# RoyiAvital/QuadraticProgramSolver

Hardware: AMD Instinct MI355X
Metric: ADMM iterations/sec (higher is better)
Workload: dtype f64

## Files before the change

quadraticprogramsolver_amd/csrc/k_loop.hip:

```cpp
#include <cstdlib>

#include "qps_kernels.h"
#include "wave_reduce.h"
#include <hip/hip_ext.h>

namespace qps {

namespace {

template <typename T> __device__ __forceinline__ T wave_sum(T v) { return wave_sum_all(v); }
__device__ __forceinline__ unsigned long long absbits(double v) { return (unsigned long long)__double_as_longlong(fabs(v)); }
__device__ __forceinline__ unsigned long long wave_max_u64(unsigned long long v) {
#pragma unroll
    for (int o = 32; o > 0; o >>= 1) { unsigned long long t = __shfl_xor(v, o, 64); v = t > v ? t : v; }
    return v;
}

template <typename T, int RB, int TRI, int THREADS>
__global__ __launch_bounds__(THREADS) void k_gemv_rows(const T* __restrict__ S, int64_t ld, const T* __restrict__ v,
                                                   T* __restrict__ out, const T* __restrict__ out0, T alpha, T beta,
                                                   int r0, int c0, int c1, BatchStride bs) {
    using V = typename VecOf<T>::type;
    if (bs.active && !bs.active[blockIdx.y]) return;
    S += (int64_t)blockIdx.y * bs.mat; v += (int64_t)blockIdx.y * bs.vin; out += (int64_t)blockIdx.y * bs.vout;
// ... 29 lines not shown
                acc[i] += ok ? ap[e] * vp[e] : T(0);
            }
        }
    }
    __shared__ T red[THREADS / 64][RB];
#pragma unroll
    for (int i = 0; i < RB; ++i) acc[i] = wave_sum(acc[i]);
    if ((tid & 63) == 0) {
#pragma unroll
        for (int i = 0; i < RB; ++i) red[tid >> 6][i] = acc[i];
    }
    __syncthreads();
    if (tid < RB) {
        T s = T(0);
#pragma unroll
        for (int w = 0; w < THREADS / 64; ++w) s += red[w][tid];
        T r = alpha * s;
        if (beta != T(0)) r += beta * out0[rb + tid];
        out[rb + tid] = r;
    }
}

constexpr int GC_RT = 32;
template <typename T>
__global__ __launch_bounds__(256) void k_gemv_cols(const T* __restrict__ S, int64_t ld, const T* __restrict__ va,
                                                   const T* __restrict__ vb, T ca, T cb, T* __restrict__ part,
                                                   int64_t part_ld, int ncols) {
    using V = typename VecOf<T>::type;
    constexpr int VN = VecOf<T>::N;
    const int c = (blockIdx.x * 256 + threadIdx.x) * VN;
    if (c >= ncols) return;
    const int rt = blockIdx.y;
    const int rbase = rt * GC_RT;
    T acc[VN];
#pragma unroll
    for (int e = 0; e < VN; ++e) acc[e] = T(0);
    const T* Sp = S + (int64_t)rbase * ld + c;
#pragma unroll 8
    for (int i = 0; i < GC_RT; ++i) {
        T w = ca * va[rbase + i];
        if (vb) w += cb * vb[rbase + i];
        typedef T NV __attribute__((ext_vector_type(VN)));
        const NV a = __builtin_nontemporal_load(reinterpret_cast<const NV*>(Sp + (int64_t)i * ld));
#pragma unroll
        for (int e = 0; e < VN; ++e) acc[e] += a[e] * w;
    }
    V o;
    T* op = reinterpret_cast<T*>(&o);
#pragma unroll
    for (int e = 0; e < VN; ++e) op[e] = acc[e];
    *reinterpret_cast<V*>(part + (int64_t)rt * part_ld + c) = o;
}

template <typename T>
__global__ __launch_bounds__(256) void k_colsum(const T* __restrict__ part, int64_t part_ld, int ntiles,
                                                const T* __restrict__ a0, T s0, const T* __restrict__ a1, T s1,
                                                T* __restrict__ out, int ncols, BatchStride bs) {
    using V = typename VecOf<T>::type;
    constexpr int VN = VecOf<T>::N;
    if (bs.active && !bs.active[blockIdx.y]) return;
    part += (int64_t)blockIdx.y * bs.mat; out += (int64_t)blockIdx.y * bs.vout;
    if (a0) a0 += (int64_t)blockIdx.y * bs.vin;
    if (a1) a1 += (int64_t)blockIdx.y * bs.vin;
    constexpr int COLS = 128 / (int)sizeof(T);
    constexpr int CL = COLS / VN;
    constexpr int TL = 256 / CL;
    const int cl = threadIdx.x % CL, tl = threadIdx.x / CL;
    const int c = blockIdx.x * COLS + cl * VN;
    T acc[VN];
#pragma unroll
    for (int e = 0; e < VN; ++e) acc[e] = T(0);
    if (c < ncols) {
        int t = tl;
        for (; t + 7 * TL < ntiles; t += 8 * TL) {
            V v[8];
#pragma unroll
            for (int j = 0; j < 8; ++j) v[j] = *reinterpret_cast<const V*>(part + (int64_t)(t + TL * j) * part_ld + c);
#pragma unroll
            for (int j = 0; j < 8; ++j) {
                const T* vp = reinterpret_cast<const T*>(&v[j]);
#pragma unroll
                for (int e = 0; e < VN; ++e) acc[e] += vp[e];
            }
        }
        for (; t < ntiles; t += TL) {
            const V v = *reinterpret_cast<const V*>(part + (int64_t)t * part_ld + c);
            const T* vp = reinterpret_cast<const T*>(&v);
#pragma unroll
            for (int e = 0; e < VN; ++e) acc[e] += vp[e];
        }
    }
    __shared__ T red[TL][COLS + 1];
#pragma unroll
    for (int e = 0; e < VN; ++e) red[tl][cl * VN + e] = acc[e];
    __syncthreads();
    constexpr int PL = 256 / COLS;
    static_assert(TL % PL == 0 && (PL == 16 || PL == 8), "slab lanes per output");
    const int o = threadIdx.x / PL, pl = threadIdx.x % PL;
    T s = T(0);
#pragma unroll
    for (int k = 0; k < TL / PL; ++k) s += red[pl * (TL / PL) + k][o];
    s = (PL == 16) ? row16_sum_last(s) : oct_sum_all(s);
    const int oc = blockIdx.x * COLS + o;
    if (pl == PL - 1 && oc < ncols) {
        T r = s;
        if (a0) r += s0 * a0[oc];
        if (a1) r += s1 * a1[oc];
        out[oc] = r;
    }
}

template <typename T>
__global__ __launch_bounds__(256) void k_admm_update(int NP, int MP, const T* __restrict__ xx, const T* __restrict__ zz,
                                                     T* __restrict__ x, T* __restrict__ xp, T* __restrict__ z,
                                                     T* __restrict__ zp, T* __restrict__ y, const T* __restrict__ l,
                                                     const T* __restrict__ u, T alpha, T rho) {
    const int i = blockIdx.x * 256 + threadIdx.x;
    const T alpha1 = T(1) - alpha, rho1 = T(1) / rho;
    if (i < NP) {
        const T xo = x[i];
        xp[i] = xo;
        x[i] = alpha * xx[i] + alpha1 * xo;
    }
    if (i < MP) {
        const T zo = z[i], yo = y[i], zt = zz[i];
        zp[i] = zo;
        T t = alpha * zt + alpha1 * zo + rho1 * yo;
        const T lo = l[i], hi = u[i];
        const T zn = t > hi ? hi : (t < lo ? lo : t);
        z[i] = zn;
        y[i] = yo + rho * (alpha * zt + alpha1 * zo - zn);
    }
}

template <typename T>
__global__ __launch_bounds__(256) void k_check_norms(int n, int m, const T* __restrict__ Ax, const T* __restrict__ Px,
                                                     const T* __restrict__ Aty, const T* __restrict__ q,
                                                     const T* __restrict__ x, const T* __restrict__ xp,
                                                     const T* __restrict__ z, const T* __restrict__ zp,
                                                     unsigned long long* __restrict__ slots, int dual_only, BatchStride bs) {
    if (bs.active && !bs.active[blockIdx.y]) return;
    {
        const int64_t on = (int64_t)blockIdx.y * bs.vin, om = (int64_t)blockIdx.y * bs.vout;
        Ax += om; z += om; zp += om; Px += on; Aty += on; q += on; x += on; xp += on; slots += (int64_t)blockIdx.y * 16;
    }
    unsigned long long v[9];
#pragma unroll
    for (int k = 0; k < 9; ++k) v[k] = 0ull;
    for (int i = blockIdx.x * 256 + threadIdx.x; i < max(n, m); i += gridDim.x * 256) {
        if (i < m && !dual_only) {
            const double ax = (double)Ax[i], zi = (double)z[i];
            v[0] = max(v[0], absbits((double)(Ax[i] - z[i])));
            v[2] = max(v[2], absbits(ax));
            v[3] = max(v[3], absbits(zi));
            v[8] = max(v[8], absbits((double)(z[i] - zp[i])));
        }
        if (i < n) {
            v[1] = max(v[1], absbits((double)(Px[i] + q[i] + Aty[i])));
            v[4] = max(v[4], absbits((double)Px[i]));
            v[5] = max(v[5], absbits((double)Aty[i]));
            v[6] = max(v[6], absbits((double)q[i]));
            if (!dual_only) v[7] = max(v[7], absbits((double)(x[i] - xp[i])));
        }
    }
#pragma unroll
    for (int k = 0; k < 9; ++k) {
        v[k] = wave_max_u64(v[k]);
        if ((threadIdx.x & 63) == 0 && v[k] != 0ull) atomicMax(&slots[k], v[k]);
    }
}

__device__ __forceinline__ double jmax(double a, double b) { return (isnan(a) || isnan(b)) ? (double)NAN : (a > b ? a : b); }

__global__ void k_check_decide(const unsigned long long* __restrict__ slots, double* __restrict__ res, CheckScalars cs,
                               const double* __restrict__ rho_arr, const double* __restrict__ rhorho_arr,
                               const int* __restrict__ active) {
    if (threadIdx.x != 0) return;
    const int b = blockIdx.x;
    if (active && !active[b]) return;
    slots += (int64_t)b * 16; res += (int64_t)b * 8;
    if (rho_arr) { cs.rho = rho_arr[b]; cs.rhorho = rhorho_arr[b]; cs.convFlag = 1; }
    double nv[9];
    for (int k = 0; k < 9; ++k) nv[k] = __longlong_as_double((long long)slots[k]);
    const double MIN_VAL_RHO = 1e-3, MAX_VAL_RHO = 1e6;
    const double normResPrim = nv[0], normResDual = nv[1];
    const double maxNormPrim = jmax(nv[2], nv[3]);
    const double maxNormDual = jmax(jmax(nv[4], nv[5]), nv[6]);
    double rhorho = cs.rhorho;
    if (cs.adptRho) {
        const double numeratorVal = normResPrim * maxNormDual;
        const double denominatorVal = normResDual * maxNormPrim;
        const double t = cs.rho * sqrt(numeratorVal / denominatorVal);
        rhorho = t > MAX_VAL_RHO ? MAX_VAL_RHO : (t < MIN_VAL_RHO ? MIN_VAL_RHO : t);
    }
    const double epsPrim = cs.epsAbs + cs.epsRel * maxNormPrim;
    const double epsDual = cs.epsAbs + cs.epsRel * maxNormDual;
    int flag = cs.convFlag;
    if ((normResPrim < epsPrim) && (normResDual < epsDual)) flag = 3;
    if ((nv[7] <= cs.epsAdmm) && (nv[8] <= cs.epsAdmm)) flag = 2;
    res[0] = normResPrim; res[1] = normResDual; res[2] = maxNormPrim; res[3] = maxNormDual;
    res[4] = rhorho; res[5] = (double)flag; res[6] = nv[7]; res[7] = nv[8];
}

template <typename T> __global__ void k_fill(T* p, int64_t n, T v) {
    int64_t i = (int64_t)blockIdx.x * 256 + threadIdx.x;
    if (i < n) p[i] = v;
}
template <typename T> __global__ void k_convert(const double* __restrict__ s, T* __restrict__ d, int64_t n) {
    int64_t i = (int64_t)blockIdx.x * 256 + threadIdx.x;
    if (i < n) d[i] = (T)s[i];
}
template <typename T> __global__ void k_convert_back(const T* __restrict__ s, double* __restrict__ d, int64_t n) {
    int64_t i = (int64_t)blockIdx.x * 256 + threadIdx.x;
    if (i < n) d[i] = (double)s[i];
}

}

static int env_int(const char* name, int dflt) { const char* e = getenv(name); return e ? atoi(e) : dflt; }

template <typename T, int RB, int TH>
static void gemv_rows_launch(hipStream_t st, const T* S, int64_t ld, const T* v, T* out, const T* out0, T alpha, T beta, int r0,
                             int r1, int c0, int c1, int tri, BatchStride bs) {
    dim3 grid((r1 - r0 + RB - 1) / RB, bs.count);
#define QPS_GR(TRI) hipLaunchKernelGGL((k_gemv_rows<T, RB, TRI, TH>), grid, dim3(TH), 0, st, S, ld, v, out, out0, alpha, beta, r0, c0, c1, bs)
    if (tri == 0) QPS_GR(0); else if (tri == 1) QPS_GR(1); else QPS_GR(2);
#undef QPS_GR
}

template <typename T>
void gemv_rows(hipStream_t st, const T* S, int64_t ld, const T* v, T* out, const T* out0, T alpha, T beta, int r0, int r1,
               int c0, int c1, int tri, BatchStride bs) {
    if (r1 <= r0) return;
    static const int wide_th = env_int("QPS_GEMV_WIDE_THREADS", 512);
    static const int wide_rb = env_int("QPS_GEMV_WIDE_RB", 2);
    const bool wide = (c1 - c0) >= 4 * 256 * VecOf<T>::N;
    if (!wide) { gemv_rows_launch<T, 4, 256>(st, S, ld, v, out, out0, alpha, beta, r0, r1, c0, c1, tri, bs); return; }
#define QPS_W(RB, TH) gemv_rows_launch<T, RB, TH>(st, S, ld, v, out, out0, alpha, beta, r0, r1, c0, c1, tri, bs)
    if (wide_th == 512) { if (wide_rb == 4) QPS_W(4, 512); else QPS_W(VecOf<T>::N == 2 ? 2 : 4, 512); }
    else if (wide_th == 256) { if (wide_rb == 4) QPS_W(4, 256); else QPS_W(VecOf<T>::N == 2 ? 2 : 4, 256); }
    else { if (wide_rb == 4) QPS_W(4, 1024); else QPS_W(VecOf<T>::N == 2 ? 2 : 4, 1024); }
#undef QPS_W
}

int gemv_cols_tiles(int nrows) { return (nrows + GC_RT - 1) / GC_RT; }

template <typename T>
int gemv_cols_partial(hipStream_t st, const T* S, int64_t ld, const T* va, const T* vb, T ca, T cb, T* part,
                      int64_t part_ld, int nrows, int ncols) {
    constexpr int VN = VecOf<T>::N;
    const int tiles = gemv_cols_tiles(nrows);
    if (tiles == 0) return 0;
    dim3 grid((ncols + 256 * VN - 1) / (256 * VN), tiles), block(256);
    hipLaunchKernelGGL((k_gemv_cols<T>), grid, block, 0, st, S, ld, va, vb, ca, cb, part, part_ld, ncols);
    return tiles;
}

template <typename T>
void colsum(hipStream_t st, const T* part, int64_t part_ld, int ntiles, const T* a0, T s0, const T* a1, T s1, T* out,
            int ncols, BatchStride bs) {
    constexpr int cols_wg = 128 / (int)sizeof(T);
    if (g_launch_timing.start) {
        const LaunchTiming lt = g_launch_timing;
        g_launch_timing = LaunchTiming();
        hipExtLaunchKernelGGL((k_colsum<T>), dim3((ncols + cols_wg - 1) / cols_wg, bs.count), dim3(256), 0, st, lt.start, lt.stop, 0, part, part_ld, ntiles, a0, s0, a1, s1, out, ncols, bs);
        return;
    }
    hipLaunchKernelGGL((k_colsum<T>), dim3((ncols + cols_wg - 1) / cols_wg, bs.count), dim3(256), 0, st, part, part_ld, ntiles, a0, s0, a1, s1, out, ncols, bs);
}

template <typename T>
void admm_update(hipStream_t st, int NP, int MP, const T* xx, const T* zz, T* x, T* xp, T* z, T* zp, T* y, const T* l,
                 const T* u, T alpha, T rho) {
    const int N = NP > MP ? NP : MP;
    hipLaunchKernelGGL((k_admm_update<T>), dim3((N + 255) / 256), dim3(256), 0, st, NP, MP, xx, zz, x, xp, z, zp, y, l, u, alpha, rho);
}

template <typename T>
void check_convergence(hipStream_t st, int n, int m, const T* Ax, const T* Px, const T* Aty, const T* q, const T* x,
                       const T* xp, const T* z, const T* zp, unsigned long long* scratch, double* res_dev, CheckScalars cs,
                       int dual_only, BatchStride bs, const double* rho_arr, const double* rhorho_arr) {
    if (!dual_only) (void)hipMemsetAsync(scratch, 0, 16 * sizeof(unsigned long long) * bs.count, st);
    const int N = n > m ? n : m;
    int blocks = (N + 255) / 256;
    if (blocks > 1024) blocks = 1024;
    if (blocks < 1) blocks = 1;
    hipLaunchKernelGGL((k_check_norms<T>), dim3(blocks, bs.count), dim3(256), 0, st, n, m, Ax, Px, Aty, q, x, xp, z, zp, scratch, dual_only, bs);
    hipLaunchKernelGGL(k_check_decide, dim3(bs.count), dim3(64), 0, st, scratch, res_dev, cs, rho_arr, rhorho_arr, bs.active);
}

template <typename T> void fill(hipStream_t st, T* p, int64_t n, T v) {
    if (n <= 0) return;
    hipLaunchKernelGGL((k_fill<T>), dim3((unsigned)((n + 255) / 256)), dim3(256), 0, st, p, n, v);
}
template <typename T> void convert_copy(hipStream_t st, const double* src, T* dst, int64_t n) {
    if (n <= 0) return;
    hipLaunchKernelGGL((k_convert<T>), dim3((unsigned)((n + 255) / 256)), dim3(256), 0, st, src, dst, n);
}
template <typename T> void convert_back(hipStream_t st, const T* src, double* dst, int64_t n) {
    if (n <= 0) return;
    hipLaunchKernelGGL((k_convert_back<T>), dim3((unsigned)((n + 255) / 256)), dim3(256), 0, st, src, dst, n);
}

#define INST(T)                                                                                                              \
    template void gemv_rows<T>(hipStream_t, const T*, int64_t, const T*, T*, const T*, T, T, int, int, int, int, int, BatchStride); \
    template int gemv_cols_partial<T>(hipStream_t, const T*, int64_t, const T*, const T*, T, T, T*, int64_t, int, int);      \
    template void colsum<T>(hipStream_t, const T*, int64_t, int, const T*, T, const T*, T, T*, int, BatchStride);            \
    template void admm_update<T>(hipStream_t, int, int, const T*, const T*, T*, T*, T*, T*, T*, const T*, const T*, T, T);   \
    template void check_convergence<T>(hipStream_t, int, int, const T*, const T*, const T*, const T*, const T*, const T*,    \
                                       const T*, const T*, unsigned long long*, double*, CheckScalars, int, BatchStride,     \
                                       const double*, const double*);                                                        \
    template void fill<T>(hipStream_t, T*, int64_t, T);                                                                      \
    template void convert_copy<T>(hipStream_t, const double*, T*, int64_t);                                                  \
    template void convert_back<T>(hipStream_t, const T*, double*, int64_t);
INST(double)
INST(float)
#undef INST

}
```

quadraticprogramsolver_amd/csrc/k_pass.hip:

```cpp
#include "k_pass_kernel.h"

namespace qps {

static int pass_threads() {
    static int th = [] { const char* e = getenv("QPS_PASS_THREADS"); int v = e ? atoi(e) : 512; return v == 1024 ? 1024 : 512; }();
    return th;
}

template <typename T> static int pass_threads_for(int NP) { return (pass_threads() == 1024 || NP > 8 * 512 * VecOf<T>::N) ? 1024 : 512; }
template <typename T> int apass_max_np() { return 8 * 1024 * VecOf<T>::N; }

template <typename T> int apass_plan(int NP, int MP, int* rows_per_wg, int count) {
    if (NP > apass_max_np<T>() || MP <= 0) { *rows_per_wg = 0; return 0; }
    const int R = 4;
    static const int total_env = [] { const char* e = getenv("QPS_PASS_WGS"); return e ? atoi(e) : 0; }();
    const int kc1 = NP <= pass_threads_for<T>(NP) * VecOf<T>::N;
    const int total = total_env > 0 ? total_env : ((kc1 && count > 1) ? 1024 : 256);
    const int target = count >= total ? 1 : total / (count < 1 ? 1 : count);
    int rpw = (MP + target - 1) / target;
    rpw = ((rpw + R - 1) / R) * R;
    *rows_per_wg = rpw;
    return (MP + rpw - 1) / rpw;
}

template <typename T, int TH>
void apass_th(hipStream_t st, bool check, const T* A, int64_t ld, int NP, int MP, const T* xx, const T* x_old, T* x_new, T* z,
              T* y, const T* l, const T* u, T alpha, T rho, T* part, T* part2, int64_t part_ld, unsigned long long* slots,
              PassBatch pb) {
    int rpw = 0;
    const int G = apass_plan<T>(NP, MP, &rpw, pb.count);
    pb.slabs = G;
    const int chunk = TH * VecOf<T>::N;
    const int kc = (NP + chunk - 1) / chunk;
#define QPS_PASS(KC, R, RC) launch_pass<T, TH, KC, R, RC, 0>(st, check, G, A, ld, NP, MP, rpw, xx, x_old, x_new, z, y, l, u, alpha, rho, part, part2, part_ld, slots, pb)
    if (TH == 512) {
        if (kc <= 1) QPS_PASS(1, 4, 4);
        else if (kc <= 2) QPS_PASS(2, 4, 4);
        else if (kc <= 4) QPS_PASS(4, 4, 2);
        else QPS_PASS(8, 2, 1);
    } else {
        if (kc <= 1) QPS_PASS(1, 4, 4);
        else if (kc <= 2) QPS_PASS(2, 4, 2);
        else if (kc <= 4) QPS_PASS(4, 2, 1);
        else QPS_PASS(8, 1, 1);
    }
#undef QPS_PASS
}

template <typename T>
void apass(hipStream_t st, bool check, const T* A, int64_t ld, int NP, int MP, const T* xx, const T* x_old, T* x_new, T* z,
           T* y, const T* l, const T* u, T alpha, T rho, T* part, T* part2, int64_t part_ld, unsigned long long* slots,
           PassBatch pb) {
    if (pass_threads_for<T>(NP) == 1024) apass_th<T, 1024>(st, check, A, ld, NP, MP, xx, x_old, x_new, z, y, l, u, alpha, rho, part, part2, part_ld, slots, pb);
    else apass_th<T, 512>(st, check, A, ld, NP, MP, xx, x_old, x_new, z, y, l, u, alpha, rho, part, part2, part_ld, slots, pb);
}

#define INST(T)                                                                                                            \
    template int apass_max_np<T>();                                                                                        \
    template int apass_plan<T>(int, int, int*, int);                                                                       \
    template void apass<T>(hipStream_t, bool, const T*, int64_t, int, int, const T*, const T*, T*, T*, T*, const T*, const T*, \
                           T, T, T*, T*, int64_t, unsigned long long*, PassBatch);
INST(double)
INST(float)
#undef INST

}
```

quadraticprogramsolver_amd/csrc/qps_dense.hip:

```cpp
#include <memory>

#include "dense_chol.h"
#include "qps_batch.h"
#include "qps_internal.h"
#include "qps_kernels.h"
#include "qps_polish.h"

namespace qps {
namespace {

template <typename T> struct DenseSolver : SolverBase {
    int NP = 0, MP = 0;
    T *A = nullptr, *P = nullptr, *q = nullptr, *l = nullptr, *u = nullptr;
    T *PI = nullptr, *AA = nullptr, *M = nullptr, *S = nullptr, *tmp = nullptr, *dinv = nullptr; int* fail = nullptr;
    T *x = nullptr, *xp = nullptr, *z = nullptr, *zp = nullptr, *y = nullptr, *xx = nullptr, *zz = nullptr, *tt = nullptr, *yv = nullptr;
    T *part = nullptr, *part2 = nullptr, *sw_part = nullptr, *Ax = nullptr, *Px = nullptr, *Aty = nullptr;
    T* At = nullptr; void* small_out = nullptr; void* small_out_host = nullptr; bool small_ok = false;
    StreamLease lease; Arena arena;
    double* stage_mat = nullptr; int64_t stage_mat_count = 0;
    int pass_slabs = 0, pass_rpw = 0;
    unsigned long long* scratch = nullptr; double* res_dev = nullptr; double* res_host = nullptr; double* stage = nullptr;
    bool have_AA = false, factor_valid = false; double fac_rho = 0, fac_sigma = 0; int fac_nb = 0;
    int nb = 2048; int part_tiles = 0; int num_factorizations = 0;
    unsigned long long* pub = nullptr; unsigned* abort_dev = nullptr; unsigned sweep_epoch = 0; bool blocked_off = false, fac_premul = false;
    bool use_blocked() const { return !blocked_off && trsv_blocked_supported<T>(NP, nb); }
    struct IterGraph { int count; const void* xa; double rho, sigma, alpha; int nb; hipGraphExec_t exec; };
    std::vector<IterGraph> graphs;
    bool graphs_disabled = false;
    void drop_graphs() { for (auto& gr : graphs) (void)hipGraphExecDestroy(gr.exec); graphs.clear(); }
    hipGraphExec_t iter_graph(int count, T* xa, T* xb, double rho, double sigma, double alpha) {
        for (auto& gr : graphs) if (gr.count == count && gr.xa == xa && gr.rho == rho && gr.sigma == sigma && gr.alpha == alpha && gr.nb == nb) return gr.exec;
        if (graphs_disabled) return nullptr;
        if (graphs.size() >= 8) drop_graphs();
        hipGraph_t graph = nullptr; hipGraphExec_t exec = nullptr;
        if (hipStreamBeginCapture(st, hipStreamCaptureModeThreadLocal) != hipSuccess) { (void)hipGetLastError(); graphs_disabled = true; return nullptr; }
        for (int k = 0; k < count; ++k) {
            colsum<T>(st, part, NP, pass_slabs, xa, (T)sigma, q, T(-1), tt, NP);
            sweeps();
            apass<T>(st, false, A, NP, NP, MP, xx, xa, xb, z, y, l, u, (T)alpha, (T)rho, part, part2, NP, scratch);
            std::swap(xa, xb);
        }
        if (hipStreamEndCapture(st, &graph) != hipSuccess || graph == nullptr) { (void)hipGetLastError(); graphs_disabled = true; return nullptr; }
        const hipError_t e = hipGraphInstantiate(&exec, graph, nullptr, nullptr, 0);
        (void)hipGraphDestroy(graph);
        if (e != hipSuccess) { (void)hipGetLastError(); graphs_disabled = true; return nullptr; }
        graphs.push_back({count, xa, rho, sigma, alpha, nb, exec});
        return exec;
    }
    int prof_iter = 0;
    int sample_lvl(int slot) const { return (prof.level == 1 && prof_iter % 50 == slot) ? 1 : 2; }
    int cat_atw, cat_colsum, cat_fwd, cat_bwd, cat_ax, cat_upd, cat_chk, cat_pass, cat_passchk, cat_sweep, cat_xsum, cat_small;

    DenseSolver(int dev, int64_t n_, int64_t m_, int dt) {
        device = dev; n = n_; m = m_; dtype = dt;
        HIPC(hipSetDevice(device));
        NP = roundup(n, 64); MP = roundup(m, 64);
        const int64_t nn = (int64_t)NP * NP;
        part_tiles = gemv_cols_tiles(MP);
        pass_slabs = apass_plan<T>(NP, MP, &pass_rpw);
        const int slabs = std::max(std::max(part_tiles, pass_slabs), 1);
        small_ok = admm_small_supported<T>((int)n, (int)m, NP, MP);
        stage_mat_count = std::max((int64_t)n * n, (int64_t)m * n);
        if (stage_mat_count > ((int64_t)1 << 20)) stage_mat_count = 0;
        auto layout = [&](Arena& ar) {
            A = ar.take<T>((int64_t)MP * NP); P = ar.take<T>(nn); q = ar.take<T>(NP); l = ar.take<T>(MP); u = ar.take<T>(MP);
            PI = ar.take<T>(nn); AA = ar.take<T>(nn); M = ar.take<T>(nn); S = ar.take<T>(nn); tmp = ar.take<T>(nn);
            dinv = ar.take<T>((int64_t)(NP / 64) * 4096); fail = ar.take<int>(4);
            x = ar.take<T>(NP); xp = ar.take<T>(NP); xx = ar.take<T>(NP); tt = ar.take<T>(NP); yv = ar.take<T>(NP);
            z = ar.take<T>(MP); zp = ar.take<T>(MP); y = ar.take<T>(MP); zz = ar.take<T>(MP);
            part = ar.take<T>((int64_t)slabs * NP);
            part2 = ar.take<T>((int64_t)slabs * NP);
            sw_part = ar.take<T>((int64_t)std::max(sweep_fused_slabs<T>(NP), 1) * NP);
            Ax = ar.take<T>(MP); Px = ar.take<T>(NP); Aty = ar.take<T>(NP);
            scratch = ar.take<unsigned long long>(16); res_dev = ar.take<double>(16);
            pub = ar.take<unsigned long long>(trsv_blocked_pub_words<T>(NP));
            abort_dev = reinterpret_cast<unsigned*>(res_dev + 14);
            stage = ar.take<double>((int64_t)NP + 2 * (int64_t)MP + 64);
            if (small_ok) { At = ar.take<T>((int64_t)NP * MP); small_out = ar.take<double>(32); }
            if (stage_mat_count > 0) stage_mat = ar.take<double>(stage_mat_count);
        };
        layout(arena);
        st = prof.st = lease.acquire(device, arena.planned());
        HandleResources& res = lease.res;
        char* const recycled = res.block; res.block = nullptr;
        arena.commit(st, recycled, res.block_bytes);
        layout(arena);
        res_host = reinterpret_cast<double*>(res.pinned);
        small_out_host = small_ok ? reinterpret_cast<char*>(res.pinned) + 16 * sizeof(double) : nullptr;
        const double s = sizeof(T);
        cat_atw = prof.category("gemv_cols(A'w)", s * ((double)m * n + m + n));
        cat_colsum = prof.category("colsum(rhs)", s * ((double)part_tiles * n + 3.0 * n));
        cat_fwd = prof.category("trsv_forward", s * ((double)n * (n + 1) / 2 + 2.0 * n));
        cat_bwd = prof.category("trsv_backward", s * ((double)n * (n + 1) / 2 + 2.0 * n));
        cat_ax = prof.category("gemv_rows(Ax~)", s * ((double)m * n + m + n));
        cat_upd = prof.category("admm_update", s * (3.0 * n + 7.0 * m));
        cat_chk = prof.category("check_convergence", s * (2.0 * m * n + (double)n * n + 4.0 * n + 4.0 * m));
        cat_pass = prof.category("apass(fused A-pass)", s * ((double)m * n + 3.0 * n + 6.0 * m));
        cat_passchk = prof.category("apass(check variant)", s * ((double)m * n + 4.0 * n + 6.0 * m));
        cat_sweep = prof.category("sweeps(fused fwd+bwd, triangle read once)", s * ((double)n * (n + 1) / 2 + 2.0 * n + (double)sweep_fused_slabs<T>(NP) * n));
        cat_xsum = prof.category("colsum(x~ slabs)", s * ((double)sweep_fused_slabs<T>(NP) * n + n));
        cat_small = prof.category("admm_small(whole loop in one launch; bytes per iteration)", s * ((double)m * n + (double)n * n) + s * (6.0 * n + 10.0 * m));
    }
    ~DenseSolver() override {
        (void)hipSetDevice(device);
        (void)hipStreamSynchronize(st);
        trsv_blocked_forget_stream(device, st);
        drop_graphs();
        prof.release_events();
        lease.res.block = arena.base; lease.res.block_bytes = arena.bytes; arena.base = nullptr;
    }

    void upload_vec(const double* h, T* d, int64_t count) { HIPC(upload_staged<T>(st, stage, h, d, count)); }
    void download_vec(const T* d, double* h, int64_t count) { HIPC(download_staged<T>(st, stage, d, h, count)); }
    void upload_matrix(const double* h, int64_t ldh, int rows, int cols, T* d, int64_t ldd) {
        if (rows <= 0 || cols <= 0) return;
        if (stage_mat && (int64_t)rows * cols <= stage_mat_count) {
            HIPC(hipMemcpy2DAsync(stage_mat, sizeof(double) * (size_t)rows, h, sizeof(double) * (size_t)ldh, sizeof(double) * (size_t)rows, (size_t)cols, hipMemcpyHostToDevice, st));
            import_colmajor<T>(st, stage_mat, rows, rows, cols, d, ldd);
            HIPC(hipStreamSynchronize(st));
            return;
        }
        upload_matrix_panels<T>(st, device, h, ldh, rows, cols, d, ldd);
    }

    DenseChol<T> chol() const { return {st, (int)n, NP, MP, P, A, PI, AA, M, S, tmp, dinv, fail}; }
    void factorize(double rho, double sigma, bool rebuild_all) {
        const bool rebuild = rebuild_all || !have_AA;
        const DenseChol<T> c = chol();
        factor_valid = false;
        c.form(sigma, rho, rebuild, rebuild);
        have_AA = true;
        c.factor(nb, 1, use_blocked());
        char ctx[128]; snprintf(ctx, sizeof ctx, "rho=%g, sigma=%g; factorisation #%d of this handle", rho, sigma, ++num_factorizations);
        int f = 0;
        c.check("P + sigma I + rho A'A", ctx, &f);
        factor_valid = true; fac_rho = rho; fac_sigma = sigma; fac_nb = nb; fac_premul = use_blocked();
    }
    bool sweep_gave_up(bool fetched = false) {
        if (!fac_premul) return false;
        unsigned* h = reinterpret_cast<unsigned*>(res_host + 14);
// ... 13 lines not shown
            chol().sweeps(nb, tt, yv, xx, sw_part, BatchStride(), {&prof, cat_sweep, sample_lvl(13), cat_xsum, sample_lvl(21), cat_fwd, cat_bwd, 2});
            return;
        }
        if (sweep_epoch >= 0xfffffff0u) {
            HIPC(hipMemsetAsync(pub, 0, sizeof(unsigned long long) * (size_t)trsv_blocked_pub_words<T>(NP), st));
            sweep_epoch = 0;
        }
        TrsvBlockedPair gate(device, st);
        { ProfLaunchScope ps(prof, cat_fwd, sample_lvl(13)); trsv_blocked<T>(st, false, S, NP, NP, nb, tt, yv, pub, ++sweep_epoch, abort_dev); }
        { ProfLaunchScope ps(prof, cat_bwd, sample_lvl(21)); trsv_blocked<T>(st, true, S, NP, NP, nb, yv, xx, pub, ++sweep_epoch, abort_dev); }
    }
    void linear_solve(double rho, double sigma) {
        {
            ProfScope ps(prof, cat_atw, 1);
            gemv_cols_partial<T>(st, A, NP, z, y, (T)rho, T(-1), part, NP, MP, NP);
        }
        {
            ProfScope ps(prof, cat_colsum, 2);
            colsum<T>(st, part, NP, part_tiles, x, (T)sigma, q, T(-1), tt, NP);
        }
        sweeps();
        {
            ProfScope ps(prof, cat_ax, 2);
            gemv_rows<T>(st, A, NP, xx, zz, nullptr, T(1), T(0), 0, MP, 0, NP, 0);
        }
    }

    void solve(double* xh, const qps_params& p, qps_info* info) override {
        HIPC(hipSetDevice(device));
        blocked_off = false;
        int gave_up = 0; double t_lost = 0;
        const double t_begin = now_s();
        while (solve_once(xh, p, info)) {
            ++gave_up; t_lost = now_s() - t_begin;
            const int lvl = prof.level; prof.reset(); prof.level = lvl;
        }
        if (info) { info->sweepGaveUp = gave_up; info->cgExplicit = 0; info->tLoop += t_lost; }
    }
    bool solve_once(double* xh, const qps_params& p, qps_info* info) {
        if (p.linsys != QPS_LINSYS_AUTO && p.linsys != QPS_LINSYS_CHOLESKY)
            throw QpsError(QPS_ERR_UNSUPPORTED, "dense handles offer QPS_LINSYS_CHOLESKY only (qps_create_csc with dense_path = 0 for the CG and the sparse L D L' plugins)");
        const double t0 = now_s();
        nb = pick_nb<T>(p.trsvBlock, NP);
        double rho = p.rho, sigma = p.sigma; const double alpha = p.alpha;
        const double epsAdmm = std::fmin(p.epsAbs, p.epsRel) * 1e-2;
        int convFlag = QPS_CONV_NUM_ITR;
        const bool reuse = p.reuseFactor && factor_valid && fac_rho == rho && fac_sigma == sigma && fac_nb == nb && fac_premul == use_blocked();
        if (!reuse) factorize(rho, sigma, !p.reuseFactor || !have_AA || fac_sigma != sigma);
        upload_vec(xh, x, n);
        HIPC(hipMemsetAsync(xp, 0, sizeof(T) * NP, st));
        HIPC(hipMemsetAsync(z, 0, sizeof(T) * std::max(MP, 64), st));
        HIPC(hipMemsetAsync(y, 0, sizeof(T) * std::max(MP, 64), st));
        HIPC(hipMemsetAsync(zp, 0, sizeof(T) * std::max(MP, 64), st));
        HIPC(hipStreamSynchronize(st));
        const double t1 = now_s();
        double rhorho = rho;
        int ii = 0, nref = 0; double tref = 0, resP = NAN, resD = NAN;
        auto finish = [&](int iterations, double t_end, int variant) {
            PolishReport pr;
            if (p.polish) polish_dense<T>(st, n, m, NP, MP, P, A, q, l, u, y, x, part, p, &pr);
            download_vec(x, xh, n);
            if (info) {
                info->convFlag = convFlag; info->iterations = iterations; info->numRefactor = nref; info->cgIterations = 0;
                info->rhoFinal = rho; info->rhoProposed = rhorho; info->resPrim = resP; info->resDual = resD;
                info->tSetup = t1 - t0; info->tLoop = t_end - t1; info->tRefactor = tref;
                info->polishFlag = pr.flag; info->polishIterations = pr.minresIterations; info->tPolish = pr.seconds;
                info->trsvBlock = nb; info->sweepVariant = variant;
            }
            return false;
        };
        if (small_ok && p.loopVariant == 0 && (NP + nb - 1) / nb == 1) {
            transpose_small<T>(st, A, NP, MP, At);
            int it = 0;
            while (it < p.numIterations) {
                {
                    ProfScope ps(prof, cat_small, 1);
                    admm_small<T>(st, (int)n, (int)m, NP, MP, it, p.numIterations, p.numItrConv, p.adptRho, rho, rhorho, sigma, alpha, p.epsAbs,
                                  p.epsRel, epsAdmm, p.fctrRho, A, At, P, S, q, l, u, x, xp, z, y, small_out);
                }
                HIPC(hipMemcpyAsync(small_out_host, small_out, admm_small_out_bytes(), hipMemcpyDeviceToHost, st));
                HIPC(hipStreamSynchronize(st));
                prof.harvest();
                int last = 0, flag = 1, need = 0; double r8[8];
                admm_small_read(small_out_host, &last, &flag, &need, r8);
                it = last; convFlag = flag; rhorho = r8[4];
                if (!std::isnan(r8[0]) || !std::isnan(r8[1])) { resP = r8[0]; resD = r8[1]; }
                if (flag != QPS_CONV_NUM_ITR) break;
                if (need && it < p.numIterations) {
                    rho = rhorho; ++nref;
                    const double ta = now_s();
                    factorize(rho, sigma, false);
                    tref += now_s() - ta;
                }
            }
            return finish(it, now_s(), 4);
        }
        const bool fused = pass_slabs > 0 && p.loopVariant != 1;
        int rhs_slabs = 0;
        static const int graph_env = [] { const char* e = getenv("QPS_GRAPH"); return e ? atoi(e) : -1; }();
        const bool use_graph = fused && prof.level == 0 && p.numItrConv >= 3 && !fac_premul && (graph_env >= 0 ? graph_env != 0 : NP <= 2048);
        for (ii = 1; ii <= p.numIterations; ++ii) {
            bool changed = false;
            if (p.adptRho && ((rhorho * p.fctrRho < rho) || (rhorho > p.fctrRho * rho))) {
                rho = rhorho; ++nref; changed = true;
                const double ta = now_s();
                factorize(rho, sigma, false);
                tref += now_s() - ta;
            }
            const bool check = (ii % p.numItrConv == 0);
            if (use_graph && !changed && !check && rhs_slabs == pass_slabs) {
                int run = std::min(p.numItrConv - ii % p.numItrConv, p.numIterations - ii + 1) & ~1;
                hipGraphExec_t ge = run >= 2 ? iter_graph(run, x, xp, rho, sigma, alpha) : nullptr;
                if (ge) {
                    HIPC(hipGraphLaunch(ge, st));
                    ii += run - 1;
                    continue;
                }
            }
            if (!fused) {
                linear_solve(rho, sigma);
                {
                    ProfScope ps(prof, cat_upd, 2);
                    admm_update<T>(st, NP, MP, xx, zz, x, xp, z, zp, y, l, u, (T)alpha, (T)rho);
                }
                if (check) {
                    ProfScope ps(prof, cat_chk, 2);
                    gemv_rows<T>(st, A, NP, x, Ax, nullptr, T(1), T(0), 0, MP, 0, NP, 0);
                    gemv_rows<T>(st, P, NP, x, Px, nullptr, T(1), T(0), 0, NP, 0, NP, 0);
                    gemv_cols_partial<T>(st, A, NP, y, nullptr, T(1), T(0), part, NP, MP, NP);
                    colsum<T>(st, part, NP, part_tiles, nullptr, T(0), nullptr, T(0), Aty, NP);
                    CheckScalars cs{p.epsAbs, p.epsRel, epsAdmm, rho, rhorho, p.adptRho, convFlag};
                    check_convergence<T>(st, (int)n, (int)m, Ax, Px, Aty, q, x, xp, z, zp, scratch, res_dev, cs);
                }
            } else {
                if (changed && rhs_slabs > 0) {
                    ProfScope ps(prof, cat_atw, 2);
                    rhs_slabs = gemv_cols_partial<T>(st, A, NP, z, y, (T)rho, T(-1), part, NP, MP, NP);
                }
                prof_iter = ii;
                {
                    ProfLaunchScope ps(prof, cat_colsum, sample_lvl(29));
                    colsum<T>(st, part, NP, rhs_slabs, x, (T)sigma, q, T(-1), tt, NP);
                }
                sweeps();
                if (check) HIPC(hipMemsetAsync(scratch, 0, 16 * sizeof(unsigned long long), st));
                {
                    const int lvl = (prof.level == 1 && (check || ii % 50 != 38)) ? 3 : 1;
                    ProfLaunchScope ps(prof, check ? cat_passchk : cat_pass, lvl);
                    apass<T>(st, check, A, NP, NP, MP, xx, x, xp, z, y, l, u, (T)alpha, (T)rho, part, part2, NP, scratch);
                }
                std::swap(x, xp);
                rhs_slabs = pass_slabs;
                if (check) {
                    ProfScope ps(prof, cat_chk, 2);
                    colsum<T>(st, part2, NP, pass_slabs, nullptr, T(0), nullptr, T(0), Aty, NP);
                    gemv_rows<T>(st, P, NP, x, Px, nullptr, T(1), T(0), 0, NP, 0, NP, 0);
                    CheckScalars cs{p.epsAbs, p.epsRel, epsAdmm, rho, rhorho, p.adptRho, convFlag};
                    check_convergence<T>(st, (int)n, (int)m, Ax, Px, Aty, q, x, xp, z, zp, scratch, res_dev, cs, 1);
                }
            }
            if (check) {
                HIPC(hipMemcpyAsync(res_host, res_dev, 15 * sizeof(double), hipMemcpyDeviceToHost, st));
                HIPC(hipStreamSynchronize(st));
                prof.harvest();
                if (sweep_gave_up(true)) return true;
                resP = res_host[0]; resD = res_host[1]; rhorho = res_host[4]; convFlag = (int)res_host[5];
                if (convFlag != QPS_CONV_NUM_ITR) break;
            }
        }
        HIPC(hipStreamSynchronize(st));
        prof.harvest();
        if (sweep_gave_up()) return true;
        return finish(ii > p.numIterations ? p.numIterations : ii, now_s(), sweep_variant());
    }
    void polish(double* xh, const double* yh, const qps_params& p, qps_polish_report* rep) override {
        HIPC(hipSetDevice(device));
        upload_vec(xh, x, n); upload_vec(yh, y, m);
        PolishReport pr;
        polish_dense<T>(st, n, m, NP, MP, P, A, q, l, u, y, x, part, p, &pr);
        download_vec(x, xh, n);
        if (rep) {
            rep->flag = pr.flag; rep->refinements = pr.refinements; rep->minresIterations = pr.minresIterations;
            rep->numActiveLower = pr.numLower; rep->numActiveUpper = pr.numUpper; rep->reserved0 = 0; rep->relres = pr.relres; rep->seconds = pr.seconds;
        }
    }
    void get_dual(double* zh, double* yh) override {
        HIPC(hipSetDevice(device));
        if (zh) download_vec(z, zh, m);
        if (yh) download_vec(y, yh, m);
    }
    void linsys_init(double rho, double sigma, int linsys, int nbreq) override {
        HIPC(hipSetDevice(device));
        if (linsys != QPS_LINSYS_AUTO && linsys != QPS_LINSYS_CHOLESKY) throw QpsError(QPS_ERR_UNSUPPORTED, "dense handles support QPS_LINSYS_CHOLESKY only");
        nb = pick_nb<T>(nbreq, NP);
        blocked_off = false;
        factorize(rho, sigma, true);
    }
    void linsys_solve(const double* xh, const double* zh, const double* yh, double rho, double sigma, int changed,
                      double* xxh, double* zzh) override {
        HIPC(hipSetDevice(device));
        if (!factor_valid && !changed) throw QpsError(QPS_ERR_BAD_ARGUMENT, "qps_linsys_solve called before qps_linsys_init");
        if (changed) factorize(rho, sigma, false);
        upload_vec(xh, x, n); upload_vec(zh, z, m); upload_vec(yh, y, m);
        linear_solve(rho, sigma);
        if (sweep_gave_up()) { factorize(rho, sigma, false); linear_solve(rho, sigma); }
        download_vec(xx, xxh, n); download_vec(zz, zzh, m);
    }
    void operator_apply(int op, const double* in, double* out, double rho, double sigma) override {
        HIPC(hipSetDevice(device));
        auto Pin = [&](T* dst) { gemv_rows<T>(st, P, NP, xx, dst, nullptr, T(1), T(0), 0, NP, 0, NP, 0); };
        auto Ain = [&](T* dst) { if (m > 0) gemv_rows<T>(st, A, NP, xx, dst, nullptr, T(1), T(0), 0, MP, 0, NP, 0); };
        auto Atv = [&](const T* v, T* dst) {
            if (m > 0) { gemv_cols_partial<T>(st, A, NP, v, nullptr, T(1), T(0), part, NP, MP, NP); colsum<T>(st, part, NP, part_tiles, nullptr, T(0), nullptr, T(0), dst, NP); }
            else HIPC(hipMemsetAsync(dst, 0, sizeof(T) * NP, st));
        };
// ... 30 lines not shown
```

quadraticprogramsolver_amd/csrc/qps_kernels.h:

```cpp
#pragma once
#ifndef QPS_NT_SLABS
#define QPS_NT_SLABS 1
#endif
#include <hip/hip_runtime.h>
#include <stdint.h>

#include <atomic>
#include <thread>

namespace qps {

constexpr int kMaxDevices = 64;
int current_device();
int device_cu_count(int device);
struct PerDeviceOnce {
    std::atomic<unsigned char> state[kMaxDevices] = {};
    template <typename F> void once(int dev, F&& f) {
        if (dev < 0 || dev >= kMaxDevices) { f(); return; }
        if (state[dev].load(std::memory_order_acquire) == 2) return;
        unsigned char expect = 0;
        if (state[dev].compare_exchange_strong(expect, 1, std::memory_order_acq_rel)) { f(); state[dev].store(2, std::memory_order_release); return; }
        while (state[dev].load(std::memory_order_acquire) != 2) std::this_thread::yield();
    }
};

struct LaunchTiming { hipEvent_t start = nullptr, stop = nullptr; };
extern thread_local LaunchTiming g_launch_timing;


struct BatchStride { int count = 1; int64_t mat = 0, vin = 0, vout = 0; const int* active = nullptr; };

template <typename T> struct VecOf;
template <> struct VecOf<double> { using type = double2; static constexpr int N = 2; };
template <> struct VecOf<float>  { using type = float4;  static constexpr int N = 4; };

template <typename T>
void gemv_rows(hipStream_t st, const T* S, int64_t ld, const T* v, T* out, const T* out0, T alpha, T beta,
               int r0, int r1, int c0, int c1, int tri, BatchStride bs = BatchStride());

template <typename T>
int gemv_cols_partial(hipStream_t st, const T* S, int64_t ld, const T* va, const T* vb, T ca, T cb,
                      T* part, int64_t part_ld, int nrows, int ncols);
int gemv_cols_tiles(int nrows);

template <typename T>
void colsum(hipStream_t st, const T* part, int64_t part_ld, int ntiles, const T* a0, T s0, const T* a1, T s1,
            T* out, int ncols, BatchStride bs = BatchStride());

template <typename T>
void admm_update(hipStream_t st, int NP, int MP, const T* xx, const T* zz, T* x, T* xp, T* z, T* zp, T* y,
                 const T* l, const T* u, T alpha, T rho);

struct CheckScalars { double epsAbs, epsRel, epsAdmm, rho, rhorho; int adptRho; int convFlag; };
template <typename T>
void check_convergence(hipStream_t st, int n, int m, const T* Ax, const T* Px, const T* Aty, const T* q, const T* x,
                       const T* xp, const T* z, const T* zp, unsigned long long* scratch , double* res_dev,
                       CheckScalars cs, int dual_only = 0, BatchStride bs = BatchStride(), const double* rho_arr = nullptr,
                       const double* rhorho_arr = nullptr);

template <typename T> int apass_plan(int NP, int MP, int* rows_per_wg, int count = 1);
template <typename T> int apass_max_np();
struct PassBatch { int count = 1; int slabs = 0; const double* rho_arr = nullptr; const int* active = nullptr; int pq_me = 0; };
template <typename T>
void apass(hipStream_t st, bool check, const T* A, int64_t ld, int NP, int MP, const T* xx, const T* x_old, T* x_new, T* z,
           T* y, const T* l, const T* u, T alpha, T rho, T* part, T* part2, int64_t part_ld, unsigned long long* slots,
           PassBatch pb = PassBatch());
template <typename T> int apass_proxqp_slabs(int NP, int MP);
template <typename T>
int apass_kkt(hipStream_t st, const T* A, int64_t ld, int NP, int MP, const T* vx, const T* vlam, const T* mask, T delta, T* out_lam,
              T* part, int64_t part_ld);
template <typename T>
int apass_proxqp(hipStream_t st, const T* G, int64_t ld, int NP, int MP, int me, const T* x, T* x_scratch, T* slack, T* dual,
                 const T* g, T rho, T* part, int64_t part_ld);

template <typename T> bool sweep_fused_supported(int NP);
template <typename T> int sweep_fused_slabs(int NP, int count = 1);
template <typename T>
int sweep_fused(hipStream_t st, const T* S, int64_t ld, int NP, const T* v, T* part, int64_t part_ld, BatchStride bs = BatchStride());

template <typename T> struct PanelArgs {
    const T* Mat = nullptr; int64_t ld = 0; int rows = 0, K = 0;
    const T* B = nullptr; int npanel = 0;
    T* out = nullptr;
    const T* q = nullptr; T *x = nullptr, *xp = nullptr;
    T *z = nullptr, *zp = nullptr, *y = nullptr, *w = nullptr; const T *l = nullptr, *u = nullptr;
    const int* active = nullptr;
    T alpha = T(0), rho = T(1), sigma = T(0);
    const T *rho_row = nullptr, *rho1_row = nullptr;
};
enum class SharedPanelOp {
    product,
    rhs,
    forward,
    backward,
    backward_x,
    rows_zy,
    rows_zy_scaled,
    start_z
};
template <typename T> void shared_panel(hipStream_t st, SharedPanelOp op, const PanelArgs<T>& a);
bool shared_panel_small(int rows, int K, size_t elem);
template <typename T>
void shared_check(hipStream_t st, int n, int m, int NP, int MP, int npanel, const T* Ax, const T* Px, const T* Aty, const T* q, const T* x, const T* xp,
                  const T* z, const T* zp, unsigned long long* slots, double* res_dev, const int* active, double epsAbs, double epsRel, double epsAdmm,
                  double rho, const int* kd = nullptr, const int* ke = nullptr);
int shared_cert_blocks(int n, int m);
template <typename T>
void shared_deltas(hipStream_t st, int n, int m, int NP, int MP, int npanel, const T* x, const T* xp, const T* y, const T* yp, const T* l, const T* u,
                   const int* active, T* dx, T* dyh);
template <typename T>
void shared_certificates(hipStream_t st, int n, int m, int NP, int MP, int npanel, const T* dx, const T* dyh, const T* Adx, const T* Pdx, const T* Atdy,
// ... 120 lines not shown
```

Measured before the change: 14620.

## Fuse Aty colsum, convergence reduction and decision into one epilogue kernel

Adds a single check-epilogue kernel that does the A'y column sum, the residual max-reductions and, through a last-block ticket counter, the convergence decision. The final block writes the results straight into mapped pinned host memory and resets the scratch slots itself. This removes the separate colsum, memset, decide kernel and device-to-host memcpy on check iterations. It relies on a grid-wide atomic ticket and self-resetting scratch that must stay consistent across calls. Separately, one pass tiling parameter changes from 2 to 4 for the kc<=4 case.

Result: no change. 14620, median of 3 (-0.0%).

```diff
diff --git a/quadraticprogramsolver_amd/csrc/k_loop.hip b/quadraticprogramsolver_amd/csrc/k_loop.hip
--- a/quadraticprogramsolver_amd/csrc/k_loop.hip
+++ b/quadraticprogramsolver_amd/csrc/k_loop.hip
@@ -105,19 +105,20 @@
     *reinterpret_cast<V*>(part + (int64_t)rt * part_ld + c) = o;
 }
 
-template <typename T>
-__global__ __launch_bounds__(256) void k_colsum(const T* __restrict__ part, int64_t part_ld, int ntiles,
-                                                const T* __restrict__ a0, T s0, const T* __restrict__ a1, T s1,
-                                                T* __restrict__ out, int ncols, BatchStride bs) {
+template <typename T> struct ColsumGeom {
+    static constexpr int VN = VecOf<T>::N;
+    static constexpr int COLS = 128 / (int)sizeof(T);
+    static constexpr int CL = COLS / VN;
+    static constexpr int TL = 256 / CL;
+    static constexpr int PL = 256 / COLS;
+    static_assert(TL % PL == 0 && (PL == 16 || PL == 8), "slab lanes per output");
+};
+template <typename T>
+__device__ __forceinline__ T colsum_workgroup(const T* __restrict__ part, int64_t part_ld, int ntiles, int ncols,
+                                              T (*red)[ColsumGeom<T>::COLS + 1]) {
     using V = typename VecOf<T>::type;
-    constexpr int VN = VecOf<T>::N;
-    if (bs.active && !bs.active[blockIdx.y]) return;
-    part += (int64_t)blockIdx.y * bs.mat; out += (int64_t)blockIdx.y * bs.vout;
-    if (a0) a0 += (int64_t)blockIdx.y * bs.vin;
-    if (a1) a1 += (int64_t)blockIdx.y * bs.vin;
-    constexpr int COLS = 128 / (int)sizeof(T);
-    constexpr int CL = COLS / VN;
-    constexpr int TL = 256 / CL;
+    using G = ColsumGeom<T>;
+    constexpr int VN = G::VN, COLS = G::COLS, CL = G::CL, TL = G::TL, PL = G::PL;
     const int cl = threadIdx.x % CL, tl = threadIdx.x / CL;
     const int c = blockIdx.x * COLS + cl * VN;
     T acc[VN];
@@ -143,19 +144,30 @@
             for (int e = 0; e < VN; ++e) acc[e] += vp[e];
         }
     }
-    __shared__ T red[TL][COLS + 1];
 #pragma unroll
     for (int e = 0; e < VN; ++e) red[tl][cl * VN + e] = acc[e];
     __syncthreads();
-    constexpr int PL = 256 / COLS;
-    static_assert(TL % PL == 0 && (PL == 16 || PL == 8), "slab lanes per output");
     const int o = threadIdx.x / PL, pl = threadIdx.x % PL;
     T s = T(0);
 #pragma unroll
     for (int k = 0; k < TL / PL; ++k) s += red[pl * (TL / PL) + k][o];
-    s = (PL == 16) ? row16_sum_last(s) : oct_sum_all(s);
-    const int oc = blockIdx.x * COLS + o;
-    if (pl == PL - 1 && oc < ncols) {
+    return (PL == 16) ? row16_sum_last(s) : oct_sum_all(s);
+}
+
+template <typename T>
+__global__ __launch_bounds__(256) void k_colsum(const T* __restrict__ part, int64_t part_ld, int ntiles,
+                                                const T* __restrict__ a0, T s0, const T* __restrict__ a1, T s1,
+                                                T* __restrict__ out, int ncols, BatchStride bs) {
+    using G = ColsumGeom<T>;
+    if (bs.active && !bs.active[blockIdx.y]) return;
+    part += (int64_t)blockIdx.y * bs.mat; out += (int64_t)blockIdx.y * bs.vout;
+    if (a0) a0 += (int64_t)blockIdx.y * bs.vin;
+    if (a1) a1 += (int64_t)blockIdx.y * bs.vin;
+    __shared__ T red[G::TL][G::COLS + 1];
+    const T s = colsum_workgroup<T>(part, part_ld, ntiles, ncols, red);
+    const int o = threadIdx.x / G::PL, pl = threadIdx.x % G::PL;
+    const int oc = blockIdx.x * G::COLS + o;
+    if (pl == G::PL - 1 && oc < ncols) {
         T r = s;
         if (a0) r += s0 * a0[oc];
         if (a1) r += s1 * a1[oc];
@@ -225,16 +237,7 @@
 
 __device__ __forceinline__ double jmax(double a, double b) { return (isnan(a) || isnan(b)) ? (double)NAN : (a > b ? a : b); }
 
-__global__ void k_check_decide(const unsigned long long* __restrict__ slots, double* __restrict__ res, CheckScalars cs,
-                               const double* __restrict__ rho_arr, const double* __restrict__ rhorho_arr,
-                               const int* __restrict__ active) {
-    if (threadIdx.x != 0) return;
-    const int b = blockIdx.x;
-    if (active && !active[b]) return;
-    slots += (int64_t)b * 16; res += (int64_t)b * 8;
-    if (rho_arr) { cs.rho = rho_arr[b]; cs.rhorho = rhorho_arr[b]; cs.convFlag = 1; }
-    double nv[9];
-    for (int k = 0; k < 9; ++k) nv[k] = __longlong_as_double((long long)slots[k]);
+__device__ __forceinline__ void check_decide(const double (&nv)[9], const CheckScalars& cs, double (&r)[8]) {
     const double MIN_VAL_RHO = 1e-3, MAX_VAL_RHO = 1e6;
     const double normResPrim = nv[0], normResDual = nv[1];
     const double maxNormPrim = jmax(nv[2], nv[3]);
@@ -251,8 +254,103 @@
     int flag = cs.convFlag;
     if ((normResPrim < epsPrim) && (normResDual < epsDual)) flag = 3;
     if ((nv[7] <= cs.epsAdmm) && (nv[8] <= cs.epsAdmm)) flag = 2;
-    res[0] = normResPrim; res[1] = normResDual; res[2] = maxNormPrim; res[3] = maxNormDual;
-    res[4] = rhorho; res[5] = (double)flag; res[6] = nv[7]; res[7] = nv[8];
+    r[0] = normResPrim; r[1] = normResDual; r[2] = maxNormPrim; r[3] = maxNormDual;
+    r[4] = rhorho; r[5] = (double)flag; r[6] = nv[7]; r[7] = nv[8];
+}
+__global__ void k_check_decide(const unsigned long long* __restrict__ slots, double* __restrict__ res, CheckScalars cs,
+                               const double* __restrict__ rho_arr, const double* __restrict__ rhorho_arr,
+                               const int* __restrict__ active) {
+    if (threadIdx.x != 0) return;
+    const int b = blockIdx.x;
+    if (active && !active[b]) return;
+    slots += (int64_t)b * 16; res += (int64_t)b * 8;
+    if (rho_arr) { cs.rho = rho_arr[b]; cs.rhorho = rhorho_arr[b]; cs.convFlag = 1; }
+    double nv[9], r[8];
+    for (int k = 0; k < 9; ++k) nv[k] = __longlong_as_double((long long)slots[k]);
+    check_decide(nv, cs, r);
+    for (int k = 0; k < 8; ++k) res[k] = r[k];
+}
+
+constexpr int kCheckTicket = 15;
+template <typename T>
+__global__ __launch_bounds__(256) void k_check_epilogue(const T* __restrict__ part, int64_t part_ld, int ntiles, T* __restrict__ Aty,
+                                                        int ncols, int n, int m, const T* __restrict__ Ax, const T* __restrict__ Px,
+                                                        const T* __restrict__ q, const T* __restrict__ x, const T* __restrict__ xp,
+                                                        const T* __restrict__ z, const T* __restrict__ zp, unsigned long long* slots,
+                                                        double* res, double* res_host, CheckScalars cs, int dual_only) {
+    using G = ColsumGeom<T>;
+    __shared__ T red[G::TL][G::COLS + 1];
+    __shared__ unsigned long long wmax[4][9];
+    const int tid = threadIdx.x;
+    const int o = tid / G::PL, pl = tid % G::PL;
+    const int oc = blockIdx.x * G::COLS + o;
+    const bool owner = pl == G::PL - 1;
+    T px = T(0), qv = T(0), dx = T(0), aty = T(0);
+    if (owner && oc < n) {
+        px = Px[oc]; qv = q[oc];
+        if (!dual_only) dx = x[oc] - xp[oc];
+        if (!part) aty = Aty[oc];
+    }
+    if (part) {
+        aty = colsum_workgroup<T>(part, part_ld, ntiles, ncols, red);
+        if (owner && oc < ncols) Aty[oc] = aty;
+    }
+    unsigned long long v[9];
+#pragma unroll
+    for (int k = 0; k < 9; ++k) v[k] = 0ull;
+    if (owner && oc < n) {
+        v[1] = absbits((double)(px + qv + aty));
+        v[4] = absbits((double)px);
+        v[5] = absbits((double)aty);
+        v[6] = absbits((double)qv);
+        if (!dual_only) v[7] = absbits((double)dx);
+    }
+    if (!dual_only) {
+        for (int i = blockIdx.x * 256 + tid; i < m; i += gridDim.x * 256) {
+            v[0] = max(v[0], absbits((double)(Ax[i] - z[i])));
+            v[2] = max(v[2], absbits((double)Ax[i]));
+            v[3] = max(v[3], absbits((double)z[i]));
+            v[8] = max(v[8], absbits((double)(z[i] - zp[i])));
+        }
+    }
+#pragma unroll
+    for (int k = 0; k < 9; ++k) {
+        const bool primal = (k == 0 || k == 2 || k == 3 || k == 7 || k == 8);
+        if (primal && dual_only) continue;
+        v[k] = wave_max_u64(v[k]);
+        if ((tid & 63) == 0) wmax[tid >> 6][k] = v[k];
+    }
+    __syncthreads();
+    if (tid < 9 && !(dual_only && (tid == 0 || tid == 2 || tid == 3 || tid == 7 || tid == 8))) {
+        unsigned long long w = wmax[0][tid];
+#pragma unroll
+        for (int k = 1; k < 4; ++k) w = max(w, wmax[k][tid]);
+        if (w != 0ull) atomicMax(&slots[tid], w);
+    }
+    asm volatile("s_waitcnt vmcnt(0)" ::: "memory");
+    __syncthreads();
+    if (tid != 0) return;
+    __builtin_amdgcn_fence(__ATOMIC_RELEASE, "agent");
+    asm volatile("s_waitcnt vmcnt(0)" ::: "memory");
+    const unsigned long long ticket = __hip_atomic_fetch_add(&slots[kCheckTicket], 1ull, __ATOMIC_RELAXED, __HIP_MEMORY_SCOPE_AGENT);
+    if (ticket != (unsigned long long)gridDim.x - 1) return;
+    __builtin_amdgcn_fence(__ATOMIC_ACQUIRE, "agent");
+    double nv[9], r[8];
+#pragma unroll
+    for (int k = 0; k < 9; ++k) nv[k] = __longlong_as_double((long long)__hip_atomic_load(&slots[k], __ATOMIC_RELAXED, __HIP_MEMORY_SCOPE_AGENT));
+    check_decide(nv, cs, r);
+    const unsigned long long give_up = reinterpret_cast<const unsigned long long*>(res)[14];
+#pragma unroll
+    for (int k = 0; k < 8; ++k) res[k] = r[k];
+    if (res_host) {
+#pragma unroll
+        for (int k = 0; k < 8; ++k) res_host[k] = r[k];
+        reinterpret_cast<unsigned long long*>(res_host)[14] = give_up;
+    }
+#pragma unroll
+    for (int k = 0; k < 9; ++k) __hip_atomic_store(&slots[k], 0ull, __ATOMIC_RELAXED, __HIP_MEMORY_SCOPE_AGENT);
+    __hip_atomic_store(&slots[kCheckTicket], 0ull, __ATOMIC_RELAXED, __HIP_MEMORY_SCOPE_AGENT);
+    __builtin_amdgcn_fence(__ATOMIC_RELEASE, "");
 }
 
 template <typename T> __global__ void k_fill(T* p, int64_t n, T v) {
@@ -332,7 +430,13 @@
 template <typename T>
 void check_convergence(hipStream_t st, int n, int m, const T* Ax, const T* Px, const T* Aty, const T* q, const T* x,
                        const T* xp, const T* z, const T* zp, unsigned long long* scratch, double* res_dev, CheckScalars cs,
-                       int dual_only, BatchStride bs, const double* rho_arr, const double* rhorho_arr) {
+                       int dual_only, BatchStride bs, const double* rho_arr, const double* rhorho_arr, const CheckEpilogue<T>* ep) {
+    if (ep) {
+        constexpr int cols_wg = 128 / (int)sizeof(T);
+        hipLaunchKernelGGL((k_check_epilogue<T>), dim3((ep->ncols + cols_wg - 1) / cols_wg), dim3(256), 0, st, ep->part, ep->part_ld, ep->ntiles, ep->Aty,
+                           ep->ncols, n, m, Ax, Px, q, x, xp, z, zp, scratch, res_dev, ep->res_host, cs, dual_only);
+        return;
+    }
     if (!dual_only) (void)hipMemsetAsync(scratch, 0, 16 * sizeof(unsigned long long) * bs.count, st);
     const int N = n > m ? n : m;
     int blocks = (N + 255) / 256;
@@ -362,7 +466,7 @@
     template void admm_update<T>(hipStream_t, int, int, const T*, const T*, T*, T*, T*, T*, T*, const T*, const T*, T, T);   \
     template void check_convergence<T>(hipStream_t, int, int, const T*, const T*, const T*, const T*, const T*, const T*,    \
                                        const T*, const T*, unsigned long long*, double*, CheckScalars, int, BatchStride,     \
-                                       const double*, const double*);                                                        \
+                                       const double*, const double*, const CheckEpilogue<T>*);                               \
     template void fill<T>(hipStream_t, T*, int64_t, T);                                                                      \
     template void convert_copy<T>(hipStream_t, const double*, T*, int64_t);                                                  \
     template void convert_back<T>(hipStream_t, const T*, double*, int64_t);
diff --git a/quadraticprogramsolver_amd/csrc/k_pass.hip b/quadraticprogramsolver_amd/csrc/k_pass.hip
--- a/quadraticprogramsolver_amd/csrc/k_pass.hip
+++ b/quadraticprogramsolver_amd/csrc/k_pass.hip
@@ -36,7 +36,7 @@
     if (TH == 512) {
         if (kc <= 1) QPS_PASS(1, 4, 4);
         else if (kc <= 2) QPS_PASS(2, 4, 4);
-        else if (kc <= 4) QPS_PASS(4, 4, 2);
+        else if (kc <= 4) QPS_PASS(4, 4, 4);
         else QPS_PASS(8, 2, 1);
     } else {
         if (kc <= 1) QPS_PASS(1, 4, 4);
diff --git a/quadraticprogramsolver_amd/csrc/qps_dense.hip b/quadraticprogramsolver_amd/csrc/qps_dense.hip
--- a/quadraticprogramsolver_amd/csrc/qps_dense.hip
+++ b/quadraticprogramsolver_amd/csrc/qps_dense.hip
@@ -20,6 +20,7 @@
     double* stage_mat = nullptr; int64_t stage_mat_count = 0;
     int pass_slabs = 0, pass_rpw = 0;
     unsigned long long* scratch = nullptr; double* res_dev = nullptr; double* res_host = nullptr; double* stage = nullptr;
+    double* res_host_dev = nullptr;
     bool have_AA = false, factor_valid = false; double fac_rho = 0, fac_sigma = 0; int fac_nb = 0;
     int nb = 2048; int part_tiles = 0; int num_factorizations = 0;
     unsigned long long* pub = nullptr; unsigned* abort_dev = nullptr; unsigned sweep_epoch = 0; bool blocked_off = false, fac_premul = false;
@@ -86,6 +87,8 @@
         arena.commit(st, recycled, res.block_bytes);
         layout(arena);
         res_host = reinterpret_cast<double*>(res.pinned);
+        HIPC(hipHostGetDevicePointer(reinterpret_cast<void**>(&res_host_dev), res_host, 0));
+        HIPC(hipMemsetAsync(scratch, 0, 16 * sizeof(unsigned long long), st));
         small_out_host = small_ok ? reinterpret_cast<char*>(res.pinned) + 16 * sizeof(double) : nullptr;
         const double s = sizeof(T);
         cat_atw = prof.category("gemv_cols(A'w)", s * ((double)m * n + m + n));
@@ -205,6 +208,7 @@
         HIPC(hipMemsetAsync(z, 0, sizeof(T) * std::max(MP, 64), st));
         HIPC(hipMemsetAsync(y, 0, sizeof(T) * std::max(MP, 64), st));
         HIPC(hipMemsetAsync(zp, 0, sizeof(T) * std::max(MP, 64), st));
+        HIPC(hipMemsetAsync(scratch, 0, 16 * sizeof(unsigned long long), st));
         HIPC(hipStreamSynchronize(st));
         const double t1 = now_s();
         double rhorho = rho;
@@ -283,7 +287,8 @@
                     gemv_cols_partial<T>(st, A, NP, y, nullptr, T(1), T(0), part, NP, MP, NP);
                     colsum<T>(st, part, NP, part_tiles, nullptr, T(0), nullptr, T(0), Aty, NP);
                     CheckScalars cs{p.epsAbs, p.epsRel, epsAdmm, rho, rhorho, p.adptRho, convFlag};
-                    check_convergence<T>(st, (int)n, (int)m, Ax, Px, Aty, q, x, xp, z, zp, scratch, res_dev, cs);
+                    const CheckEpilogue<T> ep{nullptr, 0, 0, NP, Aty, res_host_dev};
+                    check_convergence<T>(st, (int)n, (int)m, Ax, Px, Aty, q, x, xp, z, zp, scratch, res_dev, cs, 0, BatchStride(), nullptr, nullptr, &ep);
                 }
             } else {
                 if (changed && rhs_slabs > 0) {
@@ -296,7 +301,6 @@
                     colsum<T>(st, part, NP, rhs_slabs, x, (T)sigma, q, T(-1), tt, NP);
                 }
                 sweeps();
-                if (check) HIPC(hipMemsetAsync(scratch, 0, 16 * sizeof(unsigned long long), st));
                 {
                     const int lvl = (prof.level == 1 && (check || ii % 50 != 38)) ? 3 : 1;
                     ProfLaunchScope ps(prof, check ? cat_passchk : cat_pass, lvl);
@@ -306,14 +310,13 @@
                 rhs_slabs = pass_slabs;
                 if (check) {
                     ProfScope ps(prof, cat_chk, 2);
-                    colsum<T>(st, part2, NP, pass_slabs, nullptr, T(0), nullptr, T(0), Aty, NP);
                     gemv_rows<T>(st, P, NP, x, Px, nullptr, T(1), T(0), 0, NP, 0, NP, 0);
                     CheckScalars cs{p.epsAbs, p.epsRel, epsAdmm, rho, rhorho, p.adptRho, convFlag};
-                    check_convergence<T>(st, (int)n, (int)m, Ax, Px, Aty, q, x, xp, z, zp, scratch, res_dev, cs, 1);
+                    const CheckEpilogue<T> ep{part2, NP, pass_slabs, NP, Aty, res_host_dev};
+                    check_convergence<T>(st, (int)n, (int)m, Ax, Px, Aty, q, x, xp, z, zp, scratch, res_dev, cs, 1, BatchStride(), nullptr, nullptr, &ep);
                 }
             }
             if (check) {
-                HIPC(hipMemcpyAsync(res_host, res_dev, 15 * sizeof(double), hipMemcpyDeviceToHost, st));
                 HIPC(hipStreamSynchronize(st));
                 prof.harvest();
                 if (sweep_gave_up(true)) return true;
diff --git a/quadraticprogramsolver_amd/csrc/qps_kernels.h b/quadraticprogramsolver_amd/csrc/qps_kernels.h
--- a/quadraticprogramsolver_amd/csrc/qps_kernels.h
+++ b/quadraticprogramsolver_amd/csrc/qps_kernels.h
@@ -52,11 +52,12 @@
                  const T* l, const T* u, T alpha, T rho);
 
 struct CheckScalars { double epsAbs, epsRel, epsAdmm, rho, rhorho; int adptRho; int convFlag; };
+template <typename T> struct CheckEpilogue { const T* part = nullptr; int64_t part_ld = 0; int ntiles = 0; int ncols = 0; T* Aty = nullptr; double* res_host = nullptr; };
 template <typename T>
 void check_convergence(hipStream_t st, int n, int m, const T* Ax, const T* Px, const T* Aty, const T* q, const T* x,
                        const T* xp, const T* z, const T* zp, unsigned long long* scratch , double* res_dev,
                        CheckScalars cs, int dual_only = 0, BatchStride bs = BatchStride(), const double* rho_arr = nullptr,
-                       const double* rhorho_arr = nullptr);
+                       const double* rhorho_arr = nullptr, const CheckEpilogue<T>* ep = nullptr);
 
 template <typename T> int apass_plan(int NP, int MP, int* rows_per_wg, int count = 1);
 template <typename T> int apass_max_np();
```
